# mfkiwl/conan-slam

Hardware: AMD Instinct MI355X
Metric: ekf_update_steps_per_sec (higher is better)
Workload: dtype f32

## Files before the change

### conan_slam_amd/csrc/cslam_ekf.hip

```cpp
#include <hip/hip_runtime.h>

#include <algorithm>
#include <atomic>
#include <cfloat>
#include <cmath>
#include <cstdint>
#include <cstdlib>
#include <new>
#include <string>
#include <thread>
#include <vector>

#include "cslam_common.hpp"
#include "device_owners.hpp"
#include "ekf_kernels.hpp"
#include "ekf_kernels_fast.hpp"
#include "ekf_landmark_kernels.hpp"
#include "ekf_lookahead.hpp"
#include "ekf_options.hpp"
#include "ekf_pending_store.hpp"
#include "ekf_pgemm_limbs.hpp"
#include "ekf_pose_kernels.hpp"
#include "ekf_staging.hpp"
#include "host_linalg.hpp"
// ... 1629 lines not shown
        wa.w_b     = nu == 2 ? ub.pp.w : 0;
        wa.model_a = la.model.get();
        wa.model_b = la.model.get() + 1;
        wa.Gt_a    = la.fo[0].Gt.get();
        wa.u_a     = la.fo[0].U.get();
        wa.M_a     = la.fo[0].M.get();
        wa.sub_a   = la.fo[0].sub.get();
        wa.Gt_b    = la.fo[1].Gt.get();
        wa.u_b     = la.fo[1].U.get();
        wa.M_b     = la.fo[1].M.get();
        wa.sub_b   = la.fo[1].sub.get();
        wa.Y_b     = la.Y.get();
        wa.W1a     = wbase(pend.wcur) + (size_t)pend.kp * ldp;
        wa.W1b     = wa.W1a + (size_t)2 * ua.m * ldp;
        wa.ldw     = ldp;
        wa.wv_out  = ws.dWv.get();
        wa.snap    = LaSnapJob{nullptr, nullptr, nullptr, nullptr, 0};
        return wa;
    }

    int la_launch_window(bool may_hold = false)
    {
        if (la_n == 0)
        {
            return CSLAM_OK;
        }
        const int   nu = la_n;
        const LaUpd ua = la_q[0], ub = la_q[nu - 1];
        const int   ka = 2 * ua.m, kb = nu == 2 ? 2 * ub.m : 0;
        la_n = 0;
        const PredictArgs<T> held = pp;
        int rc = use_device();
        if (rc)
        {
            return rc;
        }
        if (pend.kp > 256 && (rc = flush()))
        {
            return rc;
        }
        if ((rc = ensure_k(2 * kLaMaxObs)) || (rc = ensure_w(ka + kb)) || (rc = la_ensure(pend.kp)))
        {
            return rc;
        }
        if (opt.lower && (rc = ensure_tile_list(round_up(n, kTile) / kTile)))
        {
            return rc;
        }
        const bool safe = g_engines.load() > 1;
        const unsigned n_blocks = (unsigned)(3 + ka + 2 * kb);
        const bool hold = may_hold && opt.la_hold_wide && opt.la_fused && !safe && nu == 2 && std::is_same<T, float>::value &&
                 !la.stamps.get();
        auto launch_chain = [&]() -> int {
            const LaChainArgs<T> ch = la_chain_args(ua, ub, nu, hold, la_target + n_blocks, ++la_seq);
            if (std::max(ka, kb) <= 32)
            {
                hipLaunchKernelGGL((ekf_la_chain_kernel<T, 32>), dim3(1), dim3(256), la_chain_lds<T>(32), stream_f, ch);
            }
            else
            {
                hipLaunchKernelGGL((ekf_la_chain_kernel<T, 64>), dim3(1), dim3(256), la_chain_lds<T>(64), stream_f, ch);
            }
            CSLAM_HIP_TRY(hipGetLastError());
            CSLAM_HIP_TRY(hipEventRecord(la.ev_fb.get(), stream_f));
            return CSLAM_OK;
        };
        if (!safe && (rc = launch_chain()))
        {
            return rc;
        }
        bool use_mirror = false;
        if constexpr (std::is_same<T, float>::value)
        {
            use_mirror = opt.la_mirror &&
                         (pend.kp == 0 || (pend.mirror_covers(pend.kp, n) && pend.kp <= 128 && pend.kp % 4 == 0));
        }
        const int  k8f       = round_up(pend.kp, 8);
        const bool pg_signal = !opt.la_wg_signal && !safe && pend.kp > 0 && seq.count == 0 && sizeof(T) == 4 && k8f <= 128 &&
                               opt.lower && ldp < 32768 && !limbs_take(k8f) && stream_b == stream &&
                               pend.hd_cols[pend.wcur] == 0;
        if constexpr (std::is_same<T, float>::value)
        {
            if (use_mirror)
            {
                hipLaunchKernelGGL(ekf_la_blocks_mirror_kernel, dim3(n_blocks), dim3(256), 0, stream,
                                   la_prep_args(ua, ub, nu, hold, pg_signal), la_mirror_args(ua, ub, nu, hold));
            }
        }
        if (!use_mirror)
        {
            hipLaunchKernelGGL(ekf_la_rows_kernel<T>, dim3(ka + kb), dim3(128), 0, stream, la_rows_args(ua, ub, nu, hold));
            rows_launches++;
            hipLaunchKernelGGL(ekf_la_blocks_kernel<T>, dim3(n_blocks), dim3(64), 0, stream, la_prep_args(ua, ub, nu, hold, pg_signal));
        }
        CSLAM_HIP_TRY(hipGetLastError());
        if (safe)
        {
            CSLAM_HIP_TRY(hipEventRecord(la.ev_raw.get(), stream));
            CSLAM_HIP_TRY(hipStreamWaitEvent(stream_f, la.ev_raw.get(), 0));
            if ((rc = launch_chain()))
            {
                return rc;
            }
        }
        la_target += n_blocks;
        la_sig_add = pg_signal ? n_blocks : 0u;
        rc         = flush();
        if (la_sig_add != 0)
        {
            const unsigned add = la_sig_add;
            la_sig_add         = 0;
            hipLaunchKernelGGL(ekf_la_signal_kernel, dim3(1), dim3(64), 0, stream, la.done.get(), add);
        }
        if (rc)
        {
            return rc;
        }
        bool fused = false;
        if constexpr (std::is_same<T, float>::value)
        {
            if (opt.la_fused)
            {
                fused = true;
                la_held.wa  = la_wide_args(ua, ub, nu, hold);
                la_held.k64 = opt.la_k64 && ua.m == 32 && ub.m == 32;
                la_held.wt = (opt.la_mirror && la_held.k64 && pend.kp == 0) ? la_WT.get() : nullptr;
                pend.mirror_written(la_held.wt ? ka + kb : 0, n);
                la_held.grid  = (unsigned)(round_up(n, kTile) / 32);
                la_held.valid = true;
                if (!hold && (rc = la_launch_held_wide(nullptr)))
                {
                    return rc;
                }
                last_slot = nullptr;
                last_k    = 0;
                pend.appended(ka + kb);
                sub_valid = false;
            }
        }
        if (!fused && ((rc = la_wide(ua, la.fo[0], la.ev_fb.get())) || (nu == 2 && (rc = la_wide(ub, la.fo[1], nullptr)))))
        {
            return rc;
        }
        pp = held;
        la_windows++;
        return (la.stamps.get() && la_windows == 300) ? la_report_stamps() : CSLAM_OK;
    }

    int la_report_stamps()
    {
        long long h[32];
        CSLAM_HIP_TRY(hipStreamSynchronize(stream));
        CSLAM_HIP_TRY(hipMemcpy(h, la.stamps.get(), sizeof(h), hipMemcpyDeviceToHost));
        fprintf(stderr, "[cslam la wide stamps, 10 ns ticks] ids+columns issue:%lld poll+DMA wait:%lld pht_a:%lld gain_a:%lld store+share W1_a:%lld pht_b+corr:%lld share+G_b:%lld gain_b:%lld store_b:%lld\n",
                h[17] - h[16], h[18] - h[17], h[19] - h[18], h[20] - h[19], h[21] - h[20], h[22] - h[21], h[23] - h[22],
                h[24] - h[23], h[25] - h[24]);
        fprintf(stderr, "[cslam la stamps, cycles] load+observe:%lld sums:%lld symmetrise:%lld cholesky:%lld (first half %lld) inverse:%lld outputs:%lld total:%lld\n",
                h[6] - h[0], h[7] - h[6], h[1] - h[7], h[2] - h[1], h[5] ? h[5] - h[1] : 0, h[3] - h[2], h[4] - h[3], h[4] - h[0]);
        return CSLAM_OK;
    }

    int la_drain() override { return la_n ? la_launch_window() : la_launch_held_wide(nullptr); }

    int update(const void* Zv, int m, const void* Rv, const int* idf, int batch, bool on_device) override
    {
        if (m < 0 || !Rv || (m > 0 && (!Zv || !idf)))
        {
            return fail(CSLAM_ERR_BAD_ARG, "update: bad arguments (m=%d)", m);
        }
        if (m == 0)
        {
            return CSLAM_OK;
        }
        int rc = use_device();
        if (rc)
        {
            return rc;
        }
        const T*   R    = static_cast<const T*>(Rv);
        const T*   dZ   = static_cast<const T*>(Zv);
        const int* dIdf = idf;
        if (!on_device)
        {
            const int nf = (n - 3) / 2;
            for (int i = 0; i < m; i++)
            {
                if (idf[i] < 1 || idf[i] > nf)
                {
                    return fail(CSLAM_ERR_BAD_ARG, "update: idf[%d]=%d outside 1..%d", i, idf[i], nf);
                }
            }
            if ((rc = la_launch_held_wide(nullptr)) || (rc = stage_obs(Zv, idf, m, false, &dZ, &dIdf)))
            {
                return rc;
            }
        }
        if (batch && la_eligible(m))
        {
            return la_enqueue(dZ, dIdf, m, R, on_device);
        }
        if ((rc = la_drain()))
        {
            return rc;
        }
        if (batch)
        {
            return batch_on_device(dZ, dIdf, m, R, false);
        }
        if ((rc = resolve_predict()))
        {
            return rc;
        }
        if (opt.seq_defer)
        {
            if ((rc = ensure_w(2 * m + 8)))
            {
                return rc;
            }
            if (pend.kp + 2 * m + 6 > pend.wcap && (rc = flush()))
            {
                return rc;
            }
        }
        kp_call_limit = opt.seq_defer ? pend.kp + 2 * m : 0;
        for (int i = 0; i < m; i++)
        {
            if ((rc = batch_on_device(dZ + 2 * i, dIdf + i, 1, R, opt.seq_defer != 0)))
            {
                kp_call_limit = 0;
                return rc;
            }
        }
        kp_call_limit = 0;
        if (!opt.pipeline && defer_max == 0 && (rc = flush()))
        {
            return rc;
        }
        return CSLAM_OK;
    }

    int augment(const void* Zv, int q, const void* Rv) override
    {
        if (q < 0 || !Rv || (q > 0 && !Zv))
        {
            return fail(CSLAM_ERR_BAD_ARG, "augment: bad arguments (q=%d)", q);
        }
        if (n + 2 * q > ncap)
        {
            return fail(CSLAM_ERR_CAPACITY, "augment: %d features would exceed max_landmarks=%d", (n - 3) / 2 + q, nmax);
        }
        int rc = use_device();
        if (rc)
        {
            return rc;
        }
        if (q > 0 && (rc = wait_pgemm()))
        {
            return rc;
        }
        const T* Z = static_cast<const T*>(Zv);
        const T* R = static_cast<const T*>(Rv);
        for (int i = 0; i < q; i++)
        {
            hipLaunchKernelGGL(ekf_augment_kernel<T>, dim3((n + 255) / 256), dim3(256), 0, stream, dX.get(), dP.get(),
                               dPv.get(), ldp, n, Z[2 * i], Z[2 * i + 1], R[0], R[1], R[2], R[3], opt.lower);
            CSLAM_HIP_TRY(hipGetLastError());
            n += 2;
        }
        return CSLAM_OK;
    }

    int observe_heading(double phi, int use) override
    {
        if (!use)
        {
            return CSLAM_OK;
        }
        T   sigma = (T)(((double)0.01f * kPi) / 180.0);
        int rc    = queue_step(pp, HeadingArgs<T>{1, (T)phi, sigma * sigma});
        if (rc || opt.fuse_predict)
        {
            return rc;
        }
        return launch_pose_queue();
    }

    int factor_status(int* flags, int clear) override
    {
        if (!flags)
        {
            return fail(CSLAM_ERR_BAD_ARG, "factor_status: null");
        }
        int rc = use_device();
        if (rc || (rc = la_drain()))
        {
            return rc;
        }
        CSLAM_HIP_TRY(hipMemcpyAsync(hFlags.get(), dFlags.get(), 2 * sizeof(int), hipMemcpyDeviceToHost, stream));
        CSLAM_HIP_TRY(hipStreamSynchronize(stream));
        int f = sticky_host;
        if (hFlags[0] & kFlagZeroed)
        {
            f |= CSLAM_FACTOR_ZEROED;
        }
        if (hFlags[0] & kFlagBadIdf)
        {
            f |= CSLAM_FACTOR_BAD_IDF;
// ... 740 lines not shown
```

### conan_slam_amd/csrc/cslam_ekf_batch.hip

```cpp
#include <algorithm>
#include <cstdlib>
#include <new>
#include <utility>
#include <vector>

#include "cslam_common.hpp"
#include "device_owners.hpp"
#include "ekf_kernels.hpp"
#include "ekf_kernels_fast.hpp"
#include "ekf_landmark_kernels.hpp"
#include "ekf_lookahead.hpp"
#include "ekf_options.hpp"
#include "ekf_pose_kernels.hpp"
#include "ekf_score_kernels.hpp"
#include "sim_scan_view.hpp"

using namespace cslam;

namespace cslam
{
__global__ void __launch_bounds__(128) ekf_la_rows_batch(LaBatchWin w)
{
    const LaRowsArgs<float> a = la_batch_rows(w, blockIdx.y);
    ekf_la_rows_body<float>(a);
// ... 416 lines not shown
    {
        LaBatchWin w;
        memset(&w, 0, sizeof(w));
        w.nu     = 1;
        w.ma     = m;
        w.mb     = m;
        w.Ztab   = Ztab;
        w.idftab = idftab;
        w.pp_a   = pp;
        w.pp_b   = pp;
        for (int e = 0; e < 4; e++)
        {
            w.R[e] = R[e];
        }
        pp.valid = 0;
        return window(w);
    }

    int augment_features(AugBatchArgs& za, int q, const float* R)
    {
        int rc = drain();
        if (rc)
        {
            return rc;
        }
        for (int f = 0; f < q; f++)
        {
            za.f = f;
            hipLaunchKernelGGL(ekf_augment_batch_kernel<float>, dim3((n + 255) / 256, I), dim3(256), 0, stream,
                               dX.get(), dP.get(), dPv.get(), ldp, n, za, R[0], R[1], R[2], R[3]);
            CSLAM_HIP_TRY(hipGetLastError());
            n += 2;
        }
        return CSLAM_OK;
    }

    int predict_width() const { return std::max((quirks & CSLAM_Q_PREDICT_NM4) ? (n - 4) : (n - 3), 0); }

    int max_landmarks() const { return (ncap - 3) / 2; }
    int score_blocks() const { return (std::max(max_landmarks(), 1) + 255) / 256; }

    int ensure_score()
    {
        if (dScore.get())
        {
            return CSLAM_OK;
        }
        DevBuf<double> t, p;
        DevBuf<float>  tr;
        const size_t   rows = (size_t)std::max(max_landmarks(), 1);
        int            rc   = t.alloc_zeroed((size_t)I * CSLAM_SCORE_FIELDS, stream);
        if (rc || (rc = p.alloc((size_t)I * score_blocks() * kScoreParts)) || (rc = tr.alloc(2 * rows)))
        {
            return rc;
        }
        CSLAM_HIP_TRY(hipMemsetAsync(tr.get(), 0xFF, 2 * rows * sizeof(float), stream));
        dScore      = std::move(t);
        dScoreParts = std::move(p);
        dTruth      = std::move(tr);
        return CSLAM_OK;
    }

    int score_launch(const float* xv)
    {
        const int count  = std::min(truth_count, (n - 3) / 2);
        const int blocks = (count + 255) / 256;
        if (count > 0)
        {
            hipLaunchKernelGGL(ekf_score_landmarks_batch, dim3(blocks, I), dim3(256), 0, stream, dX.get(), dPv.get(),
                               dP.get(), ldp, wregion(wcur), (long)sW(), kp, count, dTruth.get(), gate_lm,
                               dScoreParts.get());
        }
        const int record = score_calls < (long long)series_cap ? (int)score_calls : -1;
        hipLaunchKernelGGL(ekf_score_finish_batch, dim3(I), dim3(64), 0, stream, dX.get(), dPv.get(), ldp,
                           dScoreParts.get(), blocks, xv[0], xv[1], xv[2], gate_pose, dScore.get(), dSeries.get(), record, I);
        CSLAM_HIP_TRY(hipGetLastError());
        score_calls++;
        return CSLAM_OK;
    }

    int window(const LaBatchWin& w0)
    {
        LaBatchWin w = w0;
        const int  ka = 2 * w.ma, kb = w.nu == 2 ? 2 * w.mb : 0;
        const unsigned n_blocks = (unsigned)(3 + ka + 2 * kb);
        w.I        = I;
        w.n        = n;
        w.ldp      = ldp;
        w.lower    = 1;
        w.textbook = (quirks & CSLAM_Q_LOWER_CHOL_GAIN) ? 0 : 1;
        w.X        = dX.get();
        w.Pv       = dPv.get();
        w.P        = dP.get();
        w.Wp       = wregion(wcur);
        w.sW       = (long)sW();
        w.fo       = dFo.get();
        w.la       = dLa.get();
        w.wv       = dWv.get();
        w.done     = dDone.get();
        w.flags    = dFlags.get();
        w.idloc    = dIdloc.get();
        w.kp       = kp;
        w.target   = target + n_blocks;
        w.seq      = ++seq;
        w.wg_signal = opt.wg_signal;
        w.wide_direct = 0;
        w.stamps      = dStamps.get();
        w.timeout  = 20000000ull;
        if (std::max(ka, kb) <= 16)
        {
            hipLaunchKernelGGL(ekf_la_chain_batch<16>, dim3(I), dim3(256), la_chain_lds<float>(16), stream_f, w);
        }
        else if (std::max(ka, kb) <= 32)
        {
            hipLaunchKernelGGL(ekf_la_chain_batch<32>, dim3(I), dim3(256), la_chain_lds<float>(32), stream_f, w);
        }
        else
        {
            hipLaunchKernelGGL(ekf_la_chain_batch<64>, dim3(I), dim3(256), la_chain_lds<float>(64), stream_f, w);
        }
        hipLaunchKernelGGL(ekf_la_rows_batch, dim3(ka + kb, I), dim3(128), 0, stream, w);
        hipLaunchKernelGGL(ekf_la_blocks_batch, dim3(n_blocks, I), dim3(64), 0, stream, w);
        CSLAM_HIP_TRY(hipGetLastError());
        target += n_blocks;
        int rc = flush(opt.wg_signal ? 0u : n_blocks);
        if (rc)
        {
            return rc;
        }
        w.Wn = wregion(wcur);
        if (opt.wide_pairs == 1)
        {
            hipLaunchKernelGGL(ekf_la_wide_batch1, dim3(round_up(n, kTile) / 32, I), dim3(128), 0, stream, w);
        }
        else
        {
            if (opt.la_k64 && w.ma == 32 && (w.nu == 1 || w.mb == 32))
            {
                hipLaunchKernelGGL(ekf_la_wide_batch_k64, dim3(round_up(n, kTile) / 64, I), dim3(256), 0, stream, w);
            }
            else
            {
                hipLaunchKernelGGL(ekf_la_wide_batch, dim3(round_up(n, kTile) / 64, I), dim3(256), 0, stream, w);
            }
        }
        CSLAM_HIP_TRY(hipGetLastError());
        kp = ka + kb;
        windows++;
        if (dStamps.get() && windows == 300)
        {
            long long h[32];
            CSLAM_HIP_TRY(hipStreamSynchronize(stream));
            CSLAM_HIP_TRY(hipMemcpy(h, dStamps.get(), sizeof(h), hipMemcpyDeviceToHost));
            fprintf(stderr, "[cslam batch wide stamps, 10 ns ticks] ids+columns issue:%lld poll+DMA wait:%lld pht_a:%lld gain_a:%lld "
                            "store+share W1_a:%lld pht_b+corr:%lld share+G_b:%lld gain_b:%lld store_b:%lld\n",
                    h[1] - h[0], h[2] - h[1], h[3] - h[2], h[4] - h[3], h[5] - h[4], h[6] - h[5], h[7] - h[6], h[8] - h[7], h[9] - h[8]);
            std::vector<long long> wt((size_t)I * 256);
            CSLAM_HIP_TRY(hipMemcpy(wt.data(), dStamps.get() + 32, wt.size() * sizeof(long long),
                                    hipMemcpyDeviceToHost));
            const int nwg = std::min(128, round_up(n, kTile) / (32 * opt.wide_pairs));
            long long t0  = wt[0];
            for (int i = 0; i < I; i++)
            {
                for (int b = 0; b < nwg; b++)
                {
                    t0 = std::min(t0, wt[(size_t)i * 256 + 2 * b]);
                }
            }
            fprintf(stderr, "[cslam batch wide workgroups] instance 0, duration by block of rows (10 ns ticks):");
            for (int b = 0; b < nwg; b++)
            {
                fprintf(stderr, " %lld", wt[2 * b + 1] - wt[2 * b]);
            }
            fprintf(stderr, "\n");
            for (int i = 0; i < I; i++)
            {
                long long s0 = 1ll << 62, s1 = 0, e0 = 1ll << 62, e1 = 0, dsum = 0;
                for (int b = 0; b < nwg; b++)
                {
                    const long long st = wt[(size_t)i * 256 + 2 * b] - t0, en = wt[(size_t)i * 256 + 2 * b + 1] - t0;
                    s0 = std::min(s0, st), s1 = std::max(s1, st), e0 = std::min(e0, en), e1 = std::max(e1, en);
                    dsum += en - st;
                }
                fprintf(stderr, "[cslam batch wide workgroups, 10 ns ticks] instance %d: start %lld..%lld end %lld..%lld mean duration %lld\n",
                        i, s0, s1, e0, e1, dsum / nwg);
            }
        }
        return CSLAM_OK;
    }
};

extern "C" {

int cslam_ekf_batch_create(int instances, int n_landmarks, int device, int quirks, cslam_ekf_batch_t* out)
{
    return cslam_ekf_batch_create_capacity(instances, n_landmarks, n_landmarks, device, quirks, out);
}

int cslam_ekf_batch_create_capacity(int instances, int max_landmarks, int n_landmarks, int device, int quirks,
                                    cslam_ekf_batch_t* out)
{
    if (!out || instances < 1 || instances > 255 || max_landmarks < 1 || n_landmarks < 0 || n_landmarks > max_landmarks ||
        (quirks & ~CSLAM_Q_REF_EXACT))
    {
        return fail(CSLAM_ERR_BAD_ARG, "ekf_batch_create: bad arguments");
    }
    *out  = nullptr;
    int c = 0;
    if (hipGetDeviceCount(&c) != hipSuccess || c == 0)
    {
        return fail(CSLAM_ERR_NO_DEVICE, "ekf_batch_create: no HIP device (this engine has no CPU fallback)");
    }
    if (device < 0 && hipGetDevice(&device) != hipSuccess)
    {
        device = 0;
    }
    if (device >= c)
    {
        return fail(CSLAM_ERR_BAD_ARG, "ekf_batch_create: device %d of %d", device, c);
    }
    const int    ncap = 3 + 2 * max_landmarks;
    const int    ldp  = round_up(ncap, kTile);
    const size_t pb   = (size_t)instances * ldp * ldp * 4;
    if (pb >= ((size_t)1 << 32))
    {
        return fail(CSLAM_ERR_BAD_ARG, "ekf_batch_create: %d instances x %d landmarks exceed the 4 GiB covariance slab", instances,
                    max_landmarks);
    }
    cslam_ekf_batch* b = new (std::nothrow) cslam_ekf_batch(EkfBatchOptions::from_env());
    if (!b)
    {
        return fail(CSLAM_ERR_ALLOC, "ekf_batch_create: out of host memory");
    }
    b->device = device;
    b->I      = instances;
    b->n      = 3 + 2 * n_landmarks;
    b->ncap   = ncap;
    b->ldp    = ldp;
    b->quirks = quirks;
    int rc    = b->init();
    if (rc)
    {
        delete b;
        return rc;
    }
    live_engines().fetch_add(1);
    *out = b;
    return CSLAM_OK;
}

int cslam_ekf_batch_destroy(cslam_ekf_batch_t h)
{
    if (!h)
    {
        return CSLAM_OK;
    }
    live_engines().fetch_sub(1);
    delete h;
    return CSLAM_OK;
}

int cslam_ekf_batch_set_state(cslam_ekf_batch_t h, int instance, const float* X, int n, const float* P, int ldp)
{
    if (!h || !X || !P || instance < 0 || instance >= h->I || n != h->n || ldp < n)
    {
        return fail(CSLAM_ERR_BAD_ARG, "ekf_batch_set_state: bad arguments (instance %d, n %d)", instance, n);
    }
    int rc = h->use_device();
    if (rc || (rc = h->drain()) || (rc = h->sync()))
    {
        return rc;
    }
    const size_t L  = (size_t)h->ldp;
    float*       dX = h->dX.get() + instance * L;
    float*       dP = h->dP.get() + instance * L * L;
    float*       dV = h->dPv.get() + instance * 3 * L;
    CSLAM_HIP_TRY(hipMemcpyAsync(dX, X, (size_t)n * sizeof(float), hipMemcpyHostToDevice, h->stream));
    CSLAM_HIP_TRY(hipMemcpy2DAsync(dP, L * sizeof(float), P, (size_t)ldp * sizeof(float), (size_t)n * sizeof(float), (size_t)n,
                                   hipMemcpyHostToDevice, h->stream));
    CSLAM_HIP_TRY(hipMemcpyAsync(dV, dP, 3 * L * sizeof(float), hipMemcpyDeviceToDevice, h->stream));
    for (int r = 0; r < 2; r++)
    {
        CSLAM_HIP_TRY(hipMemsetAsync(h->wregion(r) + instance * h->sW(), 0, h->sW() * sizeof(float), h->stream));
    }
    CSLAM_HIP_TRY(hipMemsetAsync(h->dFlags.get() + 2 * instance, 0, 2 * sizeof(int), h->stream));
    CSLAM_HIP_TRY(hipStreamSynchronize(h->stream));
    return CSLAM_OK;
}

int cslam_ekf_batch_flush(cslam_ekf_batch_t h)
{
    if (!h)
    {
        return fail(CSLAM_ERR_BAD_ARG, "ekf_batch_flush: null handle");
    }
    int rc = h->use_device();
    if (rc || (rc = h->drain()))
    {
        return rc;
    }
    return h->flush();
}

int cslam_ekf_batch_synchronize(cslam_ekf_batch_t h)
{
    if (!h)
    {
// ... 684 lines not shown
```

### conan_slam_amd/csrc/ekf_lookahead.hpp

```cpp
#pragma once

#include <hip/hip_runtime.h>

#include "ekf_kernels.hpp"
#include "ekf_kernels_fast.hpp"

namespace cslam
{

constexpr int kLaMaxObs = 32;

__device__ inline int la_row(const int* __restrict__ idf, int s, int n)
{
    return 3 + 2 * clamp_idf(idf[s >> 1], n) - 2 + (s & 1);
}

template <typename T>
struct LaRowsArgs
{
    const T* X;
    const T* Pv;
    int      ldp, n;
    const int* idf_a;
    int        ra;
// ... 906 lines not shown
    if (tid < 3)
    {
        mo.pose[tid] = xl[tid];
    }
    if (tid < 9)
    {
        mo.pvv[tid] = s_pvv[tid];
    }
    for (int e = tid; e < mb * 10; e += 256)
    {
        mo.coef[e] = coef[e];
    }
}

constexpr int kFlagLaTimeout = 16;

template <typename T>
struct LaChainArgs
{
    FactorArgs<T>   fa, fb;
    T *             du_a, *du_b;
    LaCarryArgs<T>  ca;
    int             nu;
    const unsigned* done;
    unsigned        target;
    unsigned long long timeout;
    unsigned*       chain_done;
    unsigned        seq;
};

template <typename T, int K>
__device__ __forceinline__ void ekf_la_chain_body(const LaChainArgs<T>& a)
{
    extern __shared__ __align__(16) unsigned char la_chain_smem[];
    if (threadIdx.x < 64)
    {
        const unsigned long long t0 = __builtin_amdgcn_s_memrealtime();
        while (true)
        {
            unsigned c = threadIdx.x < 16
                             ? __hip_atomic_load(a.done + 16 * threadIdx.x, __ATOMIC_RELAXED, __HIP_MEMORY_SCOPE_AGENT)
                             : 0u;
            c += __shfl_xor(c, 1);
            c += __shfl_xor(c, 2);
            c += __shfl_xor(c, 4);
            c += __shfl_xor(c, 8);
            c = __shfl(c, 0);
            if ((int)(c - a.target) >= 0)
            {
                break;
            }
            __builtin_amdgcn_s_sleep(32);
            if (__builtin_amdgcn_s_memrealtime() - t0 > a.timeout)
            {
                if (threadIdx.x == 0)
                {
                    atomicOr(&a.fa.flags[0], kFlagLaTimeout);
                }
                break;
            }
        }
    }
    __syncthreads();
    __builtin_amdgcn_fence(__ATOMIC_ACQUIRE, "agent");
    if constexpr (std::is_same<T, float>::value)
    {
        ekf_factor_mfma_f32_body<K>(a.fa, a.du_a);
    }
    else
    {
        ekf_factor_mfma_f64_body<K>(a.fa, a.du_a);
    }
    if (a.nu == 2)
    {
        __builtin_amdgcn_fence(__ATOMIC_RELEASE, "workgroup");
        __syncthreads();
        __builtin_amdgcn_fence(__ATOMIC_ACQUIRE, "workgroup");
        ekf_la_carry_body<T>(a.ca, la_chain_smem);
        __builtin_amdgcn_fence(__ATOMIC_RELEASE, "workgroup");
        __syncthreads();
        __builtin_amdgcn_fence(__ATOMIC_ACQUIRE, "workgroup");
        if constexpr (std::is_same<T, float>::value)
        {
            ekf_factor_mfma_f32_body<K>(a.fb, a.du_b);
        }
        else
        {
            ekf_factor_mfma_f64_body<K>(a.fb, a.du_b);
        }
    }
    __builtin_amdgcn_fence(__ATOMIC_RELEASE, "agent");
    __syncthreads();
    if (threadIdx.x < 32)
    {
        __hip_atomic_store(a.chain_done + 16 * threadIdx.x, a.seq, __ATOMIC_RELAXED, __HIP_MEMORY_SCOPE_AGENT);
    }
}

template <typename T, int K>
__global__ void __launch_bounds__(256) ekf_la_chain_kernel(LaChainArgs<T> a)
{
    ekf_la_chain_body<T, K>(a);
}

struct LaSnapJob
{
    const float* Z;
    const int*   idf;
    float*       Z_out;
    int*         idf_out;
    int          m;
};

struct LaWideArgs
{
    const float* P;
    int          ldp, n, lower;
    float*       X;
    float*       Pv;
    int          nu;
    const int *  idf_a, *idf_b;
    int          ma, mb;
    int          valid_a, valid_b, w_a, w_b;
    const LaModel<float>*model_a, *model_b;
    const float *Gt_a, *u_a, *M_a, *sub_a;
    const float *Gt_b, *u_b, *M_b, *sub_b, *Y_b;
    float *      W1a, *W1b;
    int          ldw;
    float*       wv_out;
    const unsigned* chain_done;
    unsigned        seq;
    unsigned long long timeout;
    int*            flags;
    long long*      stamps;
    long long*      wg_times;
    LaSnapJob       snap;
};

__device__ __forceinline__ int la_q_of(int t, int r, int lh)
{
    return 32 * t + (r & 3) + 8 * (r >> 2) + 4 * lh;
}

template <int PAIRS = 1, int KFIX = 0, int MIRROR = 0>
__device__ __forceinline__ void ekf_la_wide_body(const LaWideArgs& a, float* wt = nullptr)
{
    static_assert(!MIRROR || (PAIRS == 1 && KFIX == 64), "the mirror belongs to the single filter's k = 64 kernel");
    __shared__ __attribute__((aligned(16))) float s_G[2][4 * 1024];
    __shared__ __attribute__((aligned(16))) float s_Y[4 * 1024];
    __shared__ __attribute__((aligned(16))) float s_model[2][512];
    __shared__ __attribute__((aligned(16))) float s_u[2][256];
    __shared__ __attribute__((aligned(16))) float s_M[2][256];
    __shared__ int   s_fx[2][kLaMaxObs];
    __shared__ float s_sum_all[PAIRS][4][32];
    const int tid = threadIdx.x, wave = __builtin_amdgcn_readfirstlane(tid >> 6), lane = tid & 63, lj = lane & 31, lh = lane >> 5;
    const int wv = wave & 1, pr = wave >> 1;
    float (*s_sum)[32] = s_sum_all[pr];
    const int row0 = (blockIdx.x * PAIRS + pr) * 32;
    const int row  = row0 + lj;
    const int rowc = row < a.n ? row : a.n - 1;
    const int ka = KFIX ? KFIX : 2 * a.ma, kb = KFIX ? KFIX : 2 * a.mb;
    int       stamp_i = 0;
    auto      stamp   = [&]() {
        if (a.stamps != nullptr && blockIdx.x == (gridDim.x >> 1) && tid == 0)
        {
            a.stamps[stamp_i++] = (long long)__builtin_amdgcn_s_memrealtime();
        }
    };
    stamp();
    if constexpr (PAIRS == 2)
    {
        if (a.wg_times != nullptr && tid == 0)
        {
            a.wg_times[2 * blockIdx.x] = (long long)__builtin_amdgcn_s_memrealtime();
        }
    }
    const int id_a = lane < a.ma ? a.idf_a[lane] : 1;
    const int id_b = (a.nu == 2 && lane < a.mb) ? a.idf_b[lane] : 1;
    float pv0 = a.Pv[(size_t)0 * a.ldp + rowc], pv1 = a.Pv[(size_t)1 * a.ldp + rowc], pv2 = a.Pv[(size_t)2 * a.ldp + rowc];
    float x   = a.X[rowc];
    if (tid < kLaMaxObs)
    {
        s_fx[0][tid] = 3 + 2 * clamp_idf(id_a, a.n) - 2;
        s_fx[1][tid] = 3 + 2 * clamp_idf(id_b, a.n) - 2;
    }
    __syncthreads();
    float pcol[2][16];
    {
        int fxv[2][8];
#pragma unroll
        for (int ub = 0; ub < 2; ub++)
        {
#pragma unroll
            for (int i = 0; i < 8; i++)
            {
                const int o = (32 * wv + (2 * i & 3) + 8 * (2 * i >> 2) + 4 * lh) >> 1;
                fxv[ub][i]  = s_fx[ub][o < kLaMaxObs ? o : 0];
            }
        }
#pragma unroll
        for (int ub = 0; ub < 2; ub++)
        {
            const int k = ub == 0 ? ka : kb;
#pragma unroll
            for (int i = 0; i < 8; i++)
            {
                const int  q  = 32 * wv + (2 * i & 3) + 8 * (2 * i >> 2) + 4 * lh;
                const bool in = q < k && (ub == 0 || a.nu == 2);
                const int  fx = in ? fxv[ub][i] : 3;
                const float va = p_sym<float>(a.P, a.ldp, rowc, fx, a.lower);
                const float vb = p_sym<float>(a.P, a.ldp, rowc, fx + 1, a.lower);
                pcol[ub][2 * i]     = in ? va : 0.f;
                pcol[ub][2 * i + 1] = in ? vb : 0.f;
            }
        }
    }
    stamp();
    if (tid == 0)
    {
        const unsigned long long t0   = __builtin_amdgcn_s_memrealtime();
        const unsigned*          word = a.chain_done + 16 * (blockIdx.x & 31u);
        while ((int)(__hip_atomic_load(word, __ATOMIC_RELAXED, __HIP_MEMORY_SCOPE_AGENT) - a.seq) < 0)
        {
            __builtin_amdgcn_s_sleep(8);
            if (__builtin_amdgcn_s_memrealtime() - t0 > a.timeout)
            {
                atomicOr(&a.flags[0], kFlagLaTimeout);
                break;
            }
        }
    }
    __syncthreads();
    __builtin_amdgcn_fence(__ATOMIC_ACQUIRE, "agent");
    typedef __attribute__((address_space(3))) void* lptr_t;
    auto dma = [&](const float* src, int count, float* dst) {
        const __amdgpu_buffer_rsrc_t rs =
            __builtin_amdgcn_make_buffer_rsrc(const_cast<float*>(src), 0, (unsigned)(count * 4), 0x00020000);
        const int pieces = (count + 255) / 256;
        int       it     = (int)(blockIdx.x & 15u);
        it               = it < pieces ? it : 0;
        for (int j = 0; j < pieces; j++, it = (it + 1 < pieces) ? it + 1 : 0)
        {
            if ((j % (2 * PAIRS)) == wave)
            {
                __builtin_amdgcn_raw_ptr_buffer_load_lds(rs, (lptr_t)(dst + it * 256), 16, (unsigned)(lane * 16),
                                                         (unsigned)(it * 1024), 0, 0);
            }
        }
    };
    dma(a.Gt_a, ka * ka, s_G[0]);
    dma(reinterpret_cast<const float*>(a.model_a), 336, s_model[0]);
    dma(a.u_a, ka, s_u[0]);
    dma(a.M_a, 3 * ka, s_M[0]);
    if (a.nu == 2)
    {
        dma(a.Y_b, ka * kb, s_Y);
        dma(reinterpret_cast<const float*>(a.model_b), 336, s_model[1]);
        dma(a.u_b, kb, s_u[1]);
        dma(a.M_b, 3 * kb, s_M[1]);
    }
    __builtin_amdgcn_s_waitcnt(0x0F70);
    __syncthreads();
    stamp();
    float* xch = s_G[1] + pr * 2048;
    float  own[16];
    float  full[32];
    auto share = [&]() {
#pragma unroll
        for (int r = 0; r < 16; r++)
        {
            xch[(wv * 16 + r) * 64 + lane] = own[r];
        }
        __syncthreads();
#pragma unroll
        for (int t = 0; t < 2; t++)
        {
#pragma unroll
            for (int r = 0; r < 16; r++)
            {
                full[t * 16 + r] = xch[(t * 16 + r) * 64 + lane];
            }
        }
    };
    auto build_own = [&](auto UB, int k, const float* sub) {
        constexpr int ub = decltype(UB)::value;
#pragma unroll
        for (int i = 0; i < 8; i++)
        {
            const int    r = 2 * i;
            const int    q = 32 * wv + (r & 3) + 8 * (r >> 2) + 4 * lh;
            const int    o = (q >> 1) < kLaMaxObs ? (q >> 1) : 0;
            const float* c = &s_model[ub][14 + o * 10];
            float        v0, v1;
            la_pht_pair<float>(c, pv0, pv1, pv2, pcol[ub][2 * i], pcol[ub][2 * i + 1], &v0, &v1);
            const bool in = (q < k) && (row < a.n);
            if (row < 3 && in)
            {
                v0 = sub[row * k + q];
                v1 = sub[row * k + q + 1];
            }
            own[r]     = in ? v0 : 0.f;
            own[r + 1] = in ? v1 : 0.f;
        }
    };
    f32x16 w1;
    auto   gain = [&](auto UB, int k) {
        constexpr int ub = decltype(UB)::value;
        const float*  Gs = s_G[ub];
        const float*  v0 = wv == 0 ? s_u[ub] : s_M[ub] + k;
        const float*  v1 = wv == 0 ? s_M[ub] : s_M[ub] + 2 * k;
        f32x16        ac0 = f32x16{0}, ac1 = f32x16{0};
        float         sa = 0.f, sb = 0.f;
        const int     cg   = 32 * wv + lj;
        const bool    cin  = cg < k;
        const int     cgc  = cin ? cg : 0;
        float g[32], e0[32], e1[32];
#pragma unroll
        for (int i = 0; i < 32; i++)
        {
            const int q  = la_q_of(i >> 4, i & 15, lh);
            const int qc = q < k ? q : 0;
            const float gv = Gs[qc * k + cgc];
            g[i]  = (q < k && cin) ? gv : 0.f;
            e0[i] = v0[qc];
            e1[i] = v1[qc];
        }
#pragma unroll
        for (int i = 0; i < 32; i++)
        {
            const float b = full[i];
            if (i & 1)
            {
                ac1 = __builtin_amdgcn_mfma_f32_32x32x2f32(g[i], b, ac1, 0, 0, 0);
            }
            else
            {
                ac0 = __builtin_amdgcn_mfma_f32_32x32x2f32(g[i], b, ac0, 0, 0, 0);
            }
            sa += b * e0[i];
            sb += b * e1[i];
        }
#pragma unroll
        for (int r = 0; r < 16; r++)
        {
            w1[r] = ac0[r] + ac1[r];
        }
        sa += __shfl_xor(sa, 32);
        sb += __shfl_xor(sb, 32);
        if (lh == 0)
        {
            s_sum[2 * wv][lj]     = sa;
            s_sum[2 * wv + 1][lj] = sb;
        }
    };
    auto store_w1 = [&](float* W, int k, bool last) {
#pragma unroll
        for (int r = 0; r < 16; r++)
        {
            const int c = la_q_of(wv, r, lh);
            if (c < k)
            {
                if (row < 3)
                {
                    if (last)
                    {
                        a.wv_out[(size_t)row * k + c] = w1[r];
                    }
                    W[(size_t)c * a.ldw + row] = 0.f;
                }
                else
                {
                    W[(size_t)c * a.ldw + row] = w1[r];
                }
            }
        }
    };
    auto store_wt = [&](int q0) {
        float* dst = wt + (size_t)row * 128 + q0 + 32 * wv + 4 * lh;
#pragma unroll
        for (int g = 0; g < 4; g++)
        {
            const float4 v = make_float4(w1[4 * g], w1[4 * g + 1], w1[4 * g + 2], w1[4 * g + 3]);
            *reinterpret_cast<float4*>(dst + 8 * g) = (row < 3) ? make_float4(0.f, 0.f, 0.f, 0.f) : v;
        }
    };
    using U0 = std::integral_constant<int, 0>;
    using U1 = std::integral_constant<int, 1>;

    if (a.valid_a && row >= 3 && row - 3 < a.w_a)
    {
        float o0, o1, o2;
        predict_stripe_col<float>(s_model[0][0], s_model[0][1], pv0, pv1, pv2, &o0, &o1, &o2);
        pv0 = o0, pv1 = o1, pv2 = o2;
    }
    build_own(U0{}, ka, a.sub_a);
    share();
    stamp();
    gain(U0{}, ka);
    stamp();
    store_w1(a.W1a, ka, a.nu == 1);
    if constexpr (MIRROR)
    {
        store_wt(0);
    }
    const float* pred_last = s_model[0];
    if (a.nu == 2)
    {
        __syncthreads();
#pragma unroll
        for (int r = 0; r < 16; r++)
        {
            own[r] = (row >= 3) ? w1[r] : 0.f;
        }
        share();
        const float xs = s_sum[0][lj], xm0 = s_sum[1][lj], xm1 = s_sum[2][lj], xm2 = s_sum[3][lj];
        if (row >= 3)
        {
            x += xs;
            pv0 -= xm0, pv1 -= xm1, pv2 -= xm2;
        }
        stamp();
        if (a.valid_b && row >= 3 && row - 3 < a.w_b)
        {
            float o0, o1, o2;
            predict_stripe_col<float>(s_model[1][0], s_model[1][1], pv0, pv1, pv2, &o0, &o1, &o2);
            pv0 = o0, pv1 = o1, pv2 = o2;
        }
        build_own(U1{}, kb, a.sub_b);
        {
            f32x16     c0 = f32x16{0}, c1 = f32x16{0};
            const int  qg  = 32 * wv + lj;
            const bool qin = qg < kb;
            const int  qgc = qin ? qg : 0;
            float      y[32];
#pragma unroll
            for (int i = 0; i < 32; i++)
            {
                const int   c  = la_q_of(i >> 4, i & 15, lh);
                const int   cc = c < ka ? c : 0;
                const float yv = s_Y[cc * kb + qgc];
                y[i]           = (c < ka && qin) ? yv : 0.f;
            }
#pragma unroll
            for (int i = 0; i < 32; i++)
            {
                if (i & 1)
                {
                    c1 = __builtin_amdgcn_mfma_f32_32x32x2f32(y[i], full[i], c1, 0, 0, 0);
                }
                else
                {
                    c0 = __builtin_amdgcn_mfma_f32_32x32x2f32(y[i], full[i], c0, 0, 0, 0);
                }
            }
            if (row >= 3)
            {
#pragma unroll
                for (int r = 0; r < 16; r++)
                {
                    own[r] -= c0[r] + c1[r];
                }
            }
        }
        stamp();
        __syncthreads();
        dma(a.Gt_b, kb * kb, s_G[1]);
        xch = s_G[0] + pr * 2048;
        share();
        __builtin_amdgcn_s_waitcnt(0x0F70);
        __syncthreads();
        stamp();
        gain(U1{}, kb);
        stamp();
        store_w1(a.W1b, kb, true);
        if constexpr (MIRROR)
        {
            store_wt(64);
        }
        pred_last = s_model[1];
    }
    __syncthreads();
    stamp();
    if constexpr (PAIRS == 2)
    {
        if (a.wg_times != nullptr && tid == 0)
        {
            a.wg_times[2 * blockIdx.x + 1] = (long long)__builtin_amdgcn_s_memrealtime();
        }
    }
    if (wv == 0 && lh == 0 && row < a.n)
    {
        const float xs = s_sum[0][lj], xm0 = s_sum[1][lj], xm1 = s_sum[2][lj], xm2 = s_sum[3][lj];
        if (row >= 3)
        {
            a.X[row]                        = x + xs;
            a.Pv[(size_t)0 * a.ldp + row] = pv0 - xm0;
            a.Pv[(size_t)1 * a.ldp + row] = pv1 - xm1;
            a.Pv[(size_t)2 * a.ldp + row] = pv2 - xm2;
        }
        else
        {
            const int   r     = row;
            const float av[3] = {pred_last[5 + r], pred_last[5 + r + 3], pred_last[5 + r + 6]};
            const float dv[3] = {xm0, xm1, xm2};
            a.X[r]            = pred_last[2 + r] + xs;
#pragma unroll
            for (int c = 0; c < 3; c++)
            {
                if (c == r)
                {
                    a.Pv[(size_t)c * a.ldp + r] = av[c] - dv[c];
                }
                else if (c < r)
                {
                    const float bcr             = pred_last[5 + c + 3 * r];
                    a.Pv[(size_t)c * a.ldp + r] = av[c] - dv[c];
                    a.Pv[(size_t)r * a.ldp + c] = bcr - dv[c];
                }
            }
        }
    }
}


namespace labatch
{
constexpr int kS = 0, kG = 4160, kGt = 8320, kV = 12480, kT = 12544, kU = 12608, kM = 12672, kSub = 12864, kXloc = 17152;
constexpr int kSlot = 17280, kFoBlock = 2 * kSlot;
constexpr int kXL = 0, kPvL = 128, kPH = 512, kPvLb = 4608, kDbb = 4864, kY = 8960, kModel = 13056, kWR = 13760;
constexpr int kModelStride = 336, kKpad = 128, kLaBlock = kWR + kKpad * 128;
constexpr int kDoneBlock = 768;
}

struct LaBatchWin
{
    int I, n, ldp, lower, textbook;
    float*  X;
    float*  Pv;
    float*  P;
    float*  Wp;
    float*  Wn;
    long    sW;
    float*  fo;
    float*  la;
    float*  wv;
    unsigned* done;
    int*      flags;
    int*      idloc;
    const float* const* Ztab;
    const int* const*   idftab;
    long zoff_a, zoff_b, ioff_a, ioff_b;
    int  ma, mb, nu;
    long long* stamps;
    int  wide_direct;
    int  wg_signal;
    PredictArgs<float> pp_a, pp_b;
    float R[4];
    int   kp;
    unsigned target, seq;
    unsigned long long timeout;
};

__device__ __forceinline__ LaRowsArgs<float> la_batch_rows(const LaBatchWin& w, int i)
{
    using namespace labatch;
    float*            la = w.la + (size_t)i * kLaBlock;
    LaRowsArgs<float> a;
    a.X     = w.X + (size_t)i * w.ldp;
    a.Pv    = w.Pv + (size_t)i * 3 * w.ldp;
    a.ldp   = w.ldp;
    a.n     = w.n;
    a.idf_a = w.idftab[i] + w.ioff_a;
    a.ra    = 2 * w.ma;
    a.idf_b = w.idftab[i] + (w.nu == 2 ? w.ioff_b : w.ioff_a);
    a.rb    = 2 * w.mb;
    a.Wp    = w.Wp + (size_t)i * w.sW;
    a.ldw   = w.ldp;
    a.kp    = w.kp;
    a.kpad  = kKpad;
    a.XL    = la + kXL;
    a.PvL   = la + kPvL;
    a.WR    = la + kWR;
    a.flags = w.flags + 2 * i;
    return a;
}

__device__ __forceinline__ LaPrepArgs<float> la_batch_prep(const LaBatchWin& w, int i)
{
    using namespace labatch;
    float*            la = w.la + (size_t)i * kLaBlock;
    float*            fo = w.fo + (size_t)i * kFoBlock;
    LaPrepArgs<float> a;
    a.P       = w.P + (size_t)i * w.ldp * w.ldp;
    a.ldp     = w.ldp;
    a.n       = w.n;
    a.lower   = w.lower;
    a.X       = w.X + (size_t)i * w.ldp;
    a.Pv      = w.Pv + (size_t)i * 3 * w.ldp;
    a.idf_a   = w.idftab[i] + w.ioff_a;
    a.idf_b   = w.idftab[i] + (w.nu == 2 ? w.ioff_b : w.ioff_a);
    a.ra      = 2 * w.ma;
    a.rb      = 2 * w.mb;
    a.pp_a    = w.pp_a;
    a.XL      = la + kXL;
    a.PvL     = la + kPvL;
    a.WR      = la + kWR;
    a.kp      = w.kp;
    a.kpad    = kKpad;
    a.sub_a   = fo + kSub;
    a.PH      = la + kPH;
    a.Dbb     = la + kDbb;
    a.PvLb    = la + kPvLb;
    a.model_a = reinterpret_cast<LaModel<float>*>(la + kModel);
    a.xloc_a  = fo + kXloc;
    a.idloc   = w.idloc + kLaMaxObs * i;
    a.done    = w.wg_signal ? w.done + (size_t)i * kDoneBlock : nullptr;
    return a;
}

__device__ __forceinline__ FactorArgs<float> la_batch_factor(const LaBatchWin& w, int i, int slot)
{
    using namespace labatch;
    float*            fo = w.fo + (size_t)i * kFoBlock + (size_t)slot * kSlot;
    FactorArgs<float> a;
    a.X   = fo + kXloc;
    a.n   = 3 + 2 * (slot == 0 ? w.ma : w.mb);
    a.Z   = w.Ztab[i] + (slot == 0 ? w.zoff_a : w.zoff_b);
    a.idf = w.idloc + kLaMaxObs * i;
    a.m   = slot == 0 ? w.ma : w.mb;
    for (int e = 0; e < 4; e++)
    {
        a.R[e] = w.R[e];
    }
    a.PHT      = nullptr;
    a.ldw      = w.ldp;
    a.dS       = fo + kS;
    a.dG       = fo + kG;
    a.dGt      = fo + kGt;
    a.dV       = fo + kV;
    a.dt       = fo + kT;
    a.flags    = w.flags + 2 * i;
    a.scratchS = nullptr;
    a.scratchG = nullptr;
    a.stamps   = nullptr;
    a.sub      = fo + kSub;
    a.dM       = fo + kM;
    a.pp       = PredictArgs<float>{0, 0.f, 0.f, 0.f, 0.f, 0.f, 0.f, 0.f, 0.f, 0};
    a.P3       = w.Pv + (size_t)i * 3 * w.ldp;
    a.ldp3     = w.ldp;
    a.pred_out = nullptr;
    a.lds_S    = 1;
    a.lds_G    = 1;
    a.textbook = w.textbook;
// ... 90 lines not shown
```

Before: 13910.

## Overlap lookahead chain poll with P column loads and streamline wide-kernel stores

```diff
diff --git a/conan_slam_amd/csrc/cslam_ekf.hip b/conan_slam_amd/csrc/cslam_ekf.hip
--- a/conan_slam_amd/csrc/cslam_ekf.hip
+++ b/conan_slam_amd/csrc/cslam_ekf.hip
@@ -1805,7 +1805,7 @@
         long long h[32];
         CSLAM_HIP_TRY(hipStreamSynchronize(stream));
         CSLAM_HIP_TRY(hipMemcpy(h, la.stamps.get(), sizeof(h), hipMemcpyDeviceToHost));
-        fprintf(stderr, "[cslam la wide stamps, 10 ns ticks] ids+columns issue:%lld poll+DMA wait:%lld pht_a:%lld gain_a:%lld store+share W1_a:%lld pht_b+corr:%lld share+G_b:%lld gain_b:%lld store_b:%lld\n",
+        fprintf(stderr, "[cslam la wide stamps, 10 ns ticks] ids+poll, columns+DMA issue:%lld load wait:%lld pht_a:%lld gain_a:%lld store+share W1_a:%lld pht_b+corr:%lld share+G_b:%lld gain_b:%lld store_b:%lld\n",
                 h[17] - h[16], h[18] - h[17], h[19] - h[18], h[20] - h[19], h[21] - h[20], h[22] - h[21], h[23] - h[22],
                 h[24] - h[23], h[25] - h[24]);
         fprintf(stderr, "[cslam la stamps, cycles] load+observe:%lld sums:%lld symmetrise:%lld cholesky:%lld (first half %lld) inverse:%lld outputs:%lld total:%lld\n",
diff --git a/conan_slam_amd/csrc/cslam_ekf_batch.hip b/conan_slam_amd/csrc/cslam_ekf_batch.hip
--- a/conan_slam_amd/csrc/cslam_ekf_batch.hip
+++ b/conan_slam_amd/csrc/cslam_ekf_batch.hip
@@ -592,7 +592,7 @@
             long long h[32];
             CSLAM_HIP_TRY(hipStreamSynchronize(stream));
             CSLAM_HIP_TRY(hipMemcpy(h, dStamps.get(), sizeof(h), hipMemcpyDeviceToHost));
-            fprintf(stderr, "[cslam batch wide stamps, 10 ns ticks] ids+columns issue:%lld poll+DMA wait:%lld pht_a:%lld gain_a:%lld "
+            fprintf(stderr, "[cslam batch wide stamps, 10 ns ticks] ids+poll, columns+DMA issue:%lld load wait:%lld pht_a:%lld gain_a:%lld "
                             "store+share W1_a:%lld pht_b+corr:%lld share+G_b:%lld gain_b:%lld store_b:%lld\n",
                     h[1] - h[0], h[2] - h[1], h[3] - h[2], h[4] - h[3], h[5] - h[4], h[6] - h[5], h[7] - h[6], h[8] - h[7], h[9] - h[8]);
             std::vector<long long> wt((size_t)I * 256);
diff --git a/conan_slam_amd/csrc/ekf_lookahead.hpp b/conan_slam_amd/csrc/ekf_lookahead.hpp
--- a/conan_slam_amd/csrc/ekf_lookahead.hpp
+++ b/conan_slam_amd/csrc/ekf_lookahead.hpp
@@ -1082,13 +1082,17 @@
     __shared__ __attribute__((aligned(16))) float s_u[2][256];
     __shared__ __attribute__((aligned(16))) float s_M[2][256];
     __shared__ int   s_fx[2][kLaMaxObs];
-    __shared__ float s_sum_all[PAIRS][4][32];
+    __shared__ __attribute__((aligned(16))) float s_sum_all[PAIRS][4][32];
+    unsigned long long* s_off = reinterpret_cast<unsigned long long*>(&s_sum_all[0][0][0]);
+    static_assert(sizeof(float) * 4 * 32 >= sizeof(unsigned long long) * 2 * kLaMaxObs, "s_off fits the row sums of one pair");
     const int tid = threadIdx.x, wave = __builtin_amdgcn_readfirstlane(tid >> 6), lane = tid & 63, lj = lane & 31, lh = lane >> 5;
     const int wv = wave & 1, pr = wave >> 1;
     float (*s_sum)[32] = s_sum_all[pr];
     const int row0 = (blockIdx.x * PAIRS + pr) * 32;
     const int row  = row0 + lj;
     const int rowc = row < a.n ? row : a.n - 1;
+    const bool pose = row0 == 0;
+    const bool body = row >= 3;
     const int ka = KFIX ? KFIX : 2 * a.ma, kb = KFIX ? KFIX : 2 * a.mb;
     int       stamp_i = 0;
     auto      stamp   = [&]() {
@@ -1105,29 +1109,62 @@
             a.wg_times[2 * blockIdx.x] = (long long)__builtin_amdgcn_s_memrealtime();
         }
     }
-    const int id_a = lane < a.ma ? a.idf_a[lane] : 1;
-    const int id_b = (a.nu == 2 && lane < a.mb) ? a.idf_b[lane] : 1;
+    const int       id_a = lane < a.ma ? a.idf_a[lane] : 1;
+    const int       id_b = (a.nu == 2 && lane < a.mb) ? a.idf_b[lane] : 1;
+    const unsigned* word = a.chain_done + 16 * (blockIdx.x & 31u);
+    unsigned        done = a.seq;
+    if (tid == 0)
+    {
+        done = __hip_atomic_load(word, __ATOMIC_RELAXED, __HIP_MEMORY_SCOPE_AGENT);
+    }
     float pv0 = a.Pv[(size_t)0 * a.ldp + rowc], pv1 = a.Pv[(size_t)1 * a.ldp + rowc], pv2 = a.Pv[(size_t)2 * a.ldp + rowc];
     float x   = a.X[rowc];
     if (tid < kLaMaxObs)
     {
-        s_fx[0][tid] = 3 + 2 * clamp_idf(id_a, a.n) - 2;
-        s_fx[1][tid] = 3 + 2 * clamp_idf(id_b, a.n) - 2;
+        const int fa = 3 + 2 * clamp_idf(id_a, a.n) - 2, fb = 3 + 2 * clamp_idf(id_b, a.n) - 2;
+        s_fx[0][tid]              = fa;
+        s_fx[1][tid]              = fb;
+        s_off[tid]                = (unsigned long long)fa * (unsigned)a.ldp;
+        s_off[kLaMaxObs + tid]    = (unsigned long long)fb * (unsigned)a.ldp;
+    }
+    if (tid == 0 && (int)(done - a.seq) < 0)
+    {
+        const unsigned long long t0 = __builtin_amdgcn_s_memrealtime();
+        while ((int)(__hip_atomic_load(word, __ATOMIC_RELAXED, __HIP_MEMORY_SCOPE_AGENT) - a.seq) < 0)
+        {
+            __builtin_amdgcn_s_sleep(8);
+            if (__builtin_amdgcn_s_memrealtime() - t0 > a.timeout)
+            {
+                atomicOr(&a.flags[0], kFlagLaTimeout);
+                break;
+            }
+        }
     }
     __syncthreads();
+    __builtin_amdgcn_fence(__ATOMIC_ACQUIRE, "agent");
     float pcol[2][16];
     {
-        int fxv[2][8];
+        int                fxv[2][8];
+        unsigned long long offv[2][8];
 #pragma unroll
         for (int ub = 0; ub < 2; ub++)
         {
 #pragma unroll
             for (int i = 0; i < 8; i++)
             {
-                const int o = (32 * wv + (2 * i & 3) + 8 * (2 * i >> 2) + 4 * lh) >> 1;
-                fxv[ub][i]  = s_fx[ub][o < kLaMaxObs ? o : 0];
-            }
-        }
+                const int o  = (32 * wv + (2 * i & 3) + 8 * (2 * i >> 2) + 4 * lh) >> 1;
+                const int oc = o < kLaMaxObs ? o : 0;
+                fxv[ub][i]   = s_fx[ub][oc];
+                offv[ub][i]  = s_off[ub * kLaMaxObs + oc];
+            }
+        }
+        const unsigned long long rowm = (unsigned long long)rowc * (unsigned)a.ldp;
+        const int                ti   = rowc >> 7;
+        auto                     psym = [&](int j, unsigned long long off) {
+            const int  tj     = j >> 7;
+            const bool direct = !a.lower || (ti > tj) || (ti == tj && rowc >= j);
+            return a.P[direct ? off + (unsigned)rowc : rowm + (unsigned)j];
+        };
 #pragma unroll
         for (int ub = 0; ub < 2; ub++)
         {
@@ -1137,58 +1174,76 @@
             {
                 const int  q  = 32 * wv + (2 * i & 3) + 8 * (2 * i >> 2) + 4 * lh;
                 const bool in = q < k && (ub == 0 || a.nu == 2);
-                const int  fx = in ? fxv[ub][i] : 3;
-                const float va = p_sym<float>(a.P, a.ldp, rowc, fx, a.lower);
-                const float vb = p_sym<float>(a.P, a.ldp, rowc, fx + 1, a.lower);
+                const float va = psym(fxv[ub][i], offv[ub][i]);
+                const float vb = psym(fxv[ub][i] + 1, offv[ub][i] + (unsigned)a.ldp);
                 pcol[ub][2 * i]     = in ? va : 0.f;
                 pcol[ub][2 * i + 1] = in ? vb : 0.f;
             }
         }
     }
-    stamp();
-    if (tid == 0)
-    {
-        const unsigned long long t0   = __builtin_amdgcn_s_memrealtime();
-        const unsigned*          word = a.chain_done + 16 * (blockIdx.x & 31u);
-        while ((int)(__hip_atomic_load(word, __ATOMIC_RELAXED, __HIP_MEMORY_SCOPE_AGENT) - a.seq) < 0)
-        {
-            __builtin_amdgcn_s_sleep(8);
-            if (__builtin_amdgcn_s_memrealtime() - t0 > a.timeout)
-            {
-                atomicOr(&a.flags[0], kFlagLaTimeout);
-                break;
-            }
-        }
-    }
-    __syncthreads();
-    __builtin_amdgcn_fence(__ATOMIC_ACQUIRE, "agent");
     typedef __attribute__((address_space(3))) void* lptr_t;
+    auto rsrc = [&](const float* src, int count) {
+        return __builtin_amdgcn_make_buffer_rsrc(const_cast<float*>(src), 0, (unsigned)(count * 4), 0x00020000);
+    };
+    auto piece = [&](const __amdgpu_buffer_rsrc_t rs, float* dst, int it) {
+        __builtin_amdgcn_raw_ptr_buffer_load_lds(rs, (lptr_t)(dst + it * 256), 16, (unsigned)(lane * 16), (unsigned)(it * 1024), 0,
+                                                 0);
+    };
     auto dma = [&](const float* src, int count, float* dst) {
-        const __amdgpu_buffer_rsrc_t rs =
-            __builtin_amdgcn_make_buffer_rsrc(const_cast<float*>(src), 0, (unsigned)(count * 4), 0x00020000);
-        const int pieces = (count + 255) / 256;
-        int       it     = (int)(blockIdx.x & 15u);
-        it               = it < pieces ? it : 0;
-        for (int j = 0; j < pieces; j++, it = (it + 1 < pieces) ? it + 1 : 0)
-        {
-            if ((j % (2 * PAIRS)) == wave)
-            {
-                __builtin_amdgcn_raw_ptr_buffer_load_lds(rs, (lptr_t)(dst + it * 256), 16, (unsigned)(lane * 16),
-                                                         (unsigned)(it * 1024), 0, 0);
-            }
+        const __amdgpu_buffer_rsrc_t rs = rsrc(src, count);
+        if constexpr (KFIX == 64)
+        {
+#pragma unroll
+            for (int jj = 0; jj < 16 / (2 * PAIRS); jj++)
+            {
+                piece(rs, dst, (int)((blockIdx.x + wave + 2 * PAIRS * jj) & 15u));
+            }
+        }
+        else
+        {
+            const int pieces = (count + 255) / 256;
+            int       it     = (int)(blockIdx.x & 15u);
+            it               = it < pieces ? it : 0;
+            for (int j = 0; j < pieces; j++, it = (it + 1 < pieces) ? it + 1 : 0)
+            {
+                if ((j % (2 * PAIRS)) == wave)
+                {
+                    piece(rs, dst, it);
+                }
+            }
+        }
+    };
+    auto dma_small = [&](int ub) {
+        const float* mdl = reinterpret_cast<const float*>(ub ? a.model_b : a.model_a);
+        const float* u   = ub ? a.u_b : a.u_a;
+        const float* M   = ub ? a.M_b : a.M_a;
+        if constexpr (KFIX == 64 && PAIRS == 1)
+        {
+            piece(rsrc(mdl, 336), s_model[ub], wave);
+            piece(rsrc(wave == 0 ? u : M, wave == 0 ? KFIX : 3 * KFIX), wave == 0 ? s_u[ub] : s_M[ub], 0);
+        }
+        else if constexpr (KFIX == 64)
+        {
+            const float* src = wave < 2 ? mdl : (wave == 2 ? u : M);
+            float*       dst = wave < 2 ? s_model[ub] : (wave == 2 ? s_u[ub] : s_M[ub]);
+            piece(rsrc(src, wave < 2 ? 336 : (wave == 2 ? KFIX : 3 * KFIX)), dst, wave < 2 ? wave : 0);
+        }
+        else
+        {
+            const int k = ub ? kb : ka;
+            dma(mdl, 336, s_model[ub]);
+            dma(u, k, s_u[ub]);
+            dma(M, 3 * k, s_M[ub]);
         }
     };
     dma(a.Gt_a, ka * ka, s_G[0]);
-    dma(reinterpret_cast<const float*>(a.model_a), 336, s_model[0]);
-    dma(a.u_a, ka, s_u[0]);
-    dma(a.M_a, 3 * ka, s_M[0]);
+    dma_small(0);
     if (a.nu == 2)
     {
         dma(a.Y_b, ka * kb, s_Y);
-        dma(reinterpret_cast<const float*>(a.model_b), 336, s_model[1]);
-        dma(a.u_b, kb, s_u[1]);
-        dma(a.M_b, 3 * kb, s_M[1]);
-    }
+        dma_small(1);
+    }
+    stamp();
     __builtin_amdgcn_s_waitcnt(0x0F70);
     __syncthreads();
     stamp();
@@ -1224,13 +1279,27 @@
             float        v0, v1;
             la_pht_pair<float>(c, pv0, pv1, pv2, pcol[ub][2 * i], pcol[ub][2 * i + 1], &v0, &v1);
             const bool in = (q < k) && (row < a.n);
-            if (row < 3 && in)
-            {
-                v0 = sub[row * k + q];
-                v1 = sub[row * k + q + 1];
-            }
             own[r]     = in ? v0 : 0.f;
             own[r + 1] = in ? v1 : 0.f;
+        }
+        if (pose)
+        {
+            const float* srow = sub + (body ? 0 : row) * k;
+            float sv[16];
+#pragma unroll
+            for (int i = 0; i < 8; i++)
+            {
+                const int r  = 2 * i;
+                const int q  = 32 * wv + (r & 3) + 8 * (r >> 2) + 4 * lh;
+                const int qc = q < k ? q : 0;
+                sv[r] = srow[qc], sv[r + 1] = srow[qc + 1];
+            }
+#pragma unroll
+            for (int r = 0; r < 16; r++)
+            {
+                const int  q    = 32 * wv + (r & 3) + 8 * (r >> 2) + 4 * lh;
+                own[r] = (!body && q < k && row < a.n) ? sv[r] : own[r];
+            }
         }
     };
     f32x16 w1;
@@ -1283,25 +1352,38 @@
             s_sum[2 * wv + 1][lj] = sb;
         }
     };
+    const unsigned wlane = (unsigned)(((32 * wv + 4 * lh) * a.ldw + row) * 4);
     auto store_w1 = [&](float* W, int k, bool last) {
+        if (pose && last)
+        {
+#pragma unroll
+            for (int r = 0; r < 16; r++)
+            {
+                const int c = la_q_of(wv, r, lh);
+                if (!body && c < k)
+                {
+                    a.wv_out[(size_t)row * k + c] = w1[r];
+                }
+            }
+        }
 #pragma unroll
         for (int r = 0; r < 16; r++)
         {
-            const int c = la_q_of(wv, r, lh);
-            if (c < k)
-            {
-                if (row < 3)
-                {
-                    if (last)
-                    {
-                        a.wv_out[(size_t)row * k + c] = w1[r];
-                    }
-                    W[(size_t)c * a.ldw + row] = 0.f;
-                }
-                else
-                {
-                    W[(size_t)c * a.ldw + row] = w1[r];
-                }
+            w1[r] = body ? w1[r] : 0.f;
+        }
+        const __amdgpu_buffer_rsrc_t rs = __builtin_amdgcn_make_buffer_rsrc(W, 0, (unsigned)(k * a.ldw * 4), 0x00020000);
+#pragma unroll
+        for (int r = 0; r < 16; r++)
+        {
+            const unsigned coff = (unsigned)(((r & 3) + 8 * (r >> 2)) * a.ldw * 4);
+            if constexpr (KFIX == 64)
+            {
+                __builtin_amdgcn_raw_buffer_store_b32(__float_as_uint(w1[r]), rs, wlane, coff, 0);
+            }
+            else
+            {
+                __builtin_amdgcn_raw_buffer_store_b32(__float_as_uint(w1[r]), rs,
+                                                      (unsigned)((la_q_of(wv, r, lh) * a.ldw + row) * 4), 0, 0);
             }
         }
     };
@@ -1310,8 +1392,7 @@
 #pragma unroll
         for (int g = 0; g < 4; g++)
         {
-            const float4 v = make_float4(w1[4 * g], w1[4 * g + 1], w1[4 * g + 2], w1[4 * g + 3]);
-            *reinterpret_cast<float4*>(dst + 8 * g) = (row < 3) ? make_float4(0.f, 0.f, 0.f, 0.f) : v;
+            *reinterpret_cast<float4*>(dst + 8 * g) = make_float4(w1[4 * g], w1[4 * g + 1], w1[4 * g + 2], w1[4 * g + 3]);
         }
     };
     using U0 = std::integral_constant<int, 0>;
@@ -1340,15 +1421,12 @@
 #pragma unroll
         for (int r = 0; r < 16; r++)
         {
-            own[r] = (row >= 3) ? w1[r] : 0.f;
+            own[r] = w1[r];
         }
         share();
         const float xs = s_sum[0][lj], xm0 = s_sum[1][lj], xm1 = s_sum[2][lj], xm2 = s_sum[3][lj];
-        if (row >= 3)
-        {
-            x += xs;
-            pv0 -= xm0, pv1 -= xm1, pv2 -= xm2;
-        }
+        x   = body ? x + xs : x;
+        pv0 = body ? pv0 - xm0 : pv0, pv1 = body ? pv1 - xm1 : pv1, pv2 = body ? pv2 - xm2 : pv2;
         stamp();
         if (a.valid_b && row >= 3 && row - 3 < a.w_b)
         {
@@ -1383,13 +1461,11 @@
                     c0 = __builtin_amdgcn_mfma_f32_32x32x2f32(y[i], full[i], c0, 0, 0, 0);
                 }
             }
-            if (row >= 3)
-            {
-#pragma unroll
-                for (int r = 0; r < 16; r++)
-                {
-                    own[r] -= c0[r] + c1[r];
-                }
+#pragma unroll
+            for (int r = 0; r < 16; r++)
+            {
+                const float corr = own[r] - (c0[r] + c1[r]);
+                own[r]           = body ? corr : own[r];
             }
         }
         stamp();
@@ -1402,7 +1478,7 @@
         stamp();
         gain(U1{}, kb);
         stamp();
-        store_w1(a.W1b, kb, true);
+            store_w1(a.W1b, kb, true);
         if constexpr (MIRROR)
         {
             store_wt(64);
@@ -1418,17 +1494,18 @@
             a.wg_times[2 * blockIdx.x + 1] = (long long)__builtin_amdgcn_s_memrealtime();
         }
     }
-    if (wv == 0 && lh == 0 && row < a.n)
-    {
-        const float xs = s_sum[0][lj], xm0 = s_sum[1][lj], xm1 = s_sum[2][lj], xm2 = s_sum[3][lj];
-        if (row >= 3)
-        {
-            a.X[row]                        = x + xs;
-            a.Pv[(size_t)0 * a.ldp + row] = pv0 - xm0;
-            a.Pv[(size_t)1 * a.ldp + row] = pv1 - xm1;
-            a.Pv[(size_t)2 * a.ldp + row] = pv2 - xm2;
-        }
-        else
+    const bool  committer = wv == 0 && lh == 0 && row < a.n;
+    const float xs = s_sum[0][lj], xm0 = s_sum[1][lj], xm1 = s_sum[2][lj], xm2 = s_sum[3][lj];
+    if (committer && body)
+    {
+        a.X[row]                      = x + xs;
+        a.Pv[(size_t)0 * a.ldp + row] = pv0 - xm0;
+        a.Pv[(size_t)1 * a.ldp + row] = pv1 - xm1;
+        a.Pv[(size_t)2 * a.ldp + row] = pv2 - xm2;
+    }
+    if (pose)
+    {
+        if (committer && !body)
         {
             const int   r     = row;
             const float av[3] = {pred_last[5 + r], pred_last[5 + r + 3], pred_last[5 + r + 6]};
```

Result: slower. 13610 (-2.2%).
